# ambicuity/Distributed-LLM-Training-and-Inference-System

Measured on AMD Instinct MI355X. Metric: tokens/sec (node) GPT-7B train, higher is better.
Workload: dtype bf16; 1 GPU; model=gpt-7b, global_batch=16, seq_len=2048, parallelism=dp1, micro_batch=16, grad_accum=1, activation_checkpoint=none, layout=planner

## Files before the change

### llmctl/ops/csrc/flash_attn_bwd.hip

```cpp
#include <cstdlib>
#include <map>
#include <mutex>

#include "attn_common.h"

namespace llmctl {
using namespace attn;
namespace {

constexpr float LOG2E = 1.4426950408889634f;
constexpr int KV_KB = 128;
constexpr int KV_QT = 64;
#ifndef LLMCTL_DKV_NBUF
#define LLMCTL_DKV_NBUF 2
#endif
constexpr int KV_NBUF = LLMCTL_DKV_NBUF;
static_assert(KV_NBUF >= 2 && KV_NBUF <= 4, "dK/dV ring depth 2-4");
constexpr int DQ_QB = 128;
constexpr int DQ_KB = 64;

struct BwdArgs {
  const unsigned short *q, *k, *v, *dout;
  const float* lse;
  const float* delta;
// ... 264 lines not shown
#pragma unroll
        for (int d = 0; d < NDB; ++d) {
          dfr[d] = tr_frag<HD>(Ds, 32 * h, d * 32, lane);
          qfr[d] = tr_frag<HD>(Qs, 32 * h, d * 32, lane);
        }
      }
      __builtin_amdgcn_sched_barrier(0);
      if (need_mask) {
#pragma unroll
        for (int gq = 0; gq < 4; ++gq) {
          const int row0 = 32 * h + 8 * gq + 4 * hh;
          int sv[4] = {0, 0, 0, 0};
          if constexpr (DOC) {
            const int4 s4 = *reinterpret_cast<const int4*>(doc_s + row0);
            sv[0] = s4.x; sv[1] = s4.y; sv[2] = s4.z; sv[3] = s4.w;
          }
#pragma unroll
          for (int j = 0; j < 4; ++j) {
            const int qq = q0 + row0 + j;
            bool ok = qq < a.S && my_key < a.S;
            if constexpr (CAUSAL) ok = ok && my_key <= qq;
            if constexpr (DOC) ok = ok && my_key >= sv[j];
            s[4 * gq + j] = ok ? s[4 * gq + j] : -INFINITY;
          }
        }
      }
      float p[16], dsv[16];
#pragma unroll
      for (int i = 0; i < 16; ++i) {
        const float pv = fast_exp2(s[i] * a.scale_log2);
        p[i] = pv;
        dsv[i] = pv * dp[i];
      }
      bf16x8_t pb[2], sb[2];
      pb[0] = to_bf16x8(p);
      pb[1] = to_bf16x8(p + 8);
      sb[0] = to_bf16x8(dsv);
      sb[1] = to_bf16x8(dsv + 8);
      if constexpr (!CAUSAL) {
#pragma unroll
        for (int d = 0; d < NDB; ++d) {
          dfr[d] = tr_frag<HD>(Ds, 32 * h, d * 32, lane);
          qfr[d] = tr_frag<HD>(Qs, 32 * h, d * 32, lane);
        }
      }
      bf16x8_t dfr1[NDB], qfr1[NDB];
#pragma unroll
      for (int d = 0; d < NDB; ++d) {
        dfr1[d] = tr_frag<HD>(Ds, 32 * h + 16, d * 32, lane);
        qfr1[d] = tr_frag<HD>(Qs, 32 * h + 16, d * 32, lane);
      }
      dvdk_step<NDB>(dv, dk, dfr, qfr, pb[0], sb[0]);
      dvdk_step<NDB>(dv, dk, dfr1, qfr1, pb[1], sb[1]);
    }
  };
  for (int t = 0; t < ntiles; t += NB) {
    step(std::integral_constant<int, 0>{}, t);
    if (t + 1 < ntiles) step(std::integral_constant<int, 1>{}, t + 1);
    if constexpr (NB >= 3)
      if (t + 2 < ntiles) step(std::integral_constant<int, 2 % NB>{}, t + 2);
    if constexpr (NB >= 4)
      if (t + 3 < ntiles) step(std::integral_constant<int, 3 % NB>{}, t + 3);
  }
#pragma unroll
  for (int d = 0; d < NDB; ++d) asm volatile("s_nop 7\n\ts_nop 7" : "+a"(dk[d]), "+a"(dv[d]));
  if (my_key < a.S) {
    const long tok = (long)b * a.S + my_key;
    unsigned short* dkp = a.dk + tok * a.dk_st + (long)hk * HD;
    unsigned short* dvp = a.dv + tok * a.dv_st + (long)hk * HD;
    const float *cr = nullptr, *sr = nullptr;
    if (a.cos_t != nullptr) {
      const long p = a.rope_pos ? (long)a.rope_pos[tok] : tok % a.rope_S;
      cr = a.cos_t + p * (HD / 2);
      sr = a.sin_t + p * (HD / 2);
    }
    store_row<HD>(dkp, dk, a.scale, hh, cr, sr);
    store_row<HD>(dvp, dv, 1.f, hh, nullptr, nullptr);
  }
}

using s2_t = __attribute__((ext_vector_type(2))) unsigned int;

__device__ __forceinline__ bf16x8_t words8(unsigned w0, unsigned w1, unsigned w2, unsigned w3) {
  using u4 = __attribute__((ext_vector_type(4))) unsigned;
  return __builtin_bit_cast(bf16x8_t, u4{w0, w1, w2, w3});
}

__device__ __forceinline__ void mfma_v(f32x16& acc, bf16x8_t a, bf16x8_t b) {
  asm volatile("v_mfma_f32_32x32x16_bf16 %0, %1, %2, %0" : "+v"(acc) : "v"(a), "a"(b) : "memory");
}

__device__ __forceinline__ void x_step(f32x16& acc_s, f32x16& acc_d, bf16x8_t a_s, bf16x8_t b_s, bf16x8_t a_d,
                                       bf16x8_t b_d, float s0, float s1, float d0, float d1, float c, unsigned& pw,
                                       unsigned& dw) {
  float t0, t1, p0, p1;
  asm volatile(
      "v_mul_f32 %[t0], %[c], %[s0]\n\t"
      "v_mul_f32 %[t1], %[c], %[s1]\n\t"
      "v_mfma_f32_32x32x16_bf16 %[as], %[xs], %[ys], %[as]\n\t"
      "v_exp_f32 %[p0], %[t0]\n\t"
      "v_exp_f32 %[p1], %[t1]\n\t"
      "v_mfma_f32_32x32x16_bf16 %[ad], %[xd], %[yd], %[ad]\n\t"
      "v_mul_f32 %[t0], %[p0], %[d0]\n\t"
      "v_mul_f32 %[t1], %[p1], %[d1]\n\t"
      "v_cvt_pk_bf16_f32 %[pw], %[p0], %[p1]\n\t"
      "v_cvt_pk_bf16_f32 %[dw], %[t0], %[t1]"
      : [as] "+v"(acc_s), [ad] "+v"(acc_d), [t0] "=&v"(t0), [t1] "=&v"(t1), [p0] "=&v"(p0), [p1] "=&v"(p1),
        [pw] "=&v"(pw), [dw] "=&v"(dw)
      : [xs] "v"(a_s), [ys] "a"(b_s), [xd] "v"(a_d), [yd] "a"(b_d), [s0] "v"(s0), [s1] "v"(s1), [d0] "v"(d0),
        [d1] "v"(d1), [c] "s"(c)
      : "memory");
}

__device__ __forceinline__ void y_step(f32x16& dv, f32x16& dk, bf16x8_t da, bf16x8_t qa, bf16x8_t p, bf16x8_t ds,
                                       float s0, float s1, float d0, float d1, float c, unsigned& pw, unsigned& dw) {
  float t0, t1, p0, p1;
  asm volatile(
      "v_mul_f32 %[t0], %[c], %[s0]\n\t"
      "v_mul_f32 %[t1], %[c], %[s1]\n\t"
      "v_mfma_f32_32x32x16_bf16 %[dv], %[da], %[p], %[dv]\n\t"
      "v_exp_f32 %[p0], %[t0]\n\t"
      "v_exp_f32 %[p1], %[t1]\n\t"
      "v_mfma_f32_32x32x16_bf16 %[dk], %[qa], %[ds], %[dk]\n\t"
      "v_mul_f32 %[t0], %[p0], %[d0]\n\t"
      "v_mul_f32 %[t1], %[p1], %[d1]\n\t"
      "v_cvt_pk_bf16_f32 %[pw], %[p0], %[p1]\n\t"
      "v_cvt_pk_bf16_f32 %[dw], %[t0], %[t1]"
      : [dv] "+a"(dv), [dk] "+a"(dk), [t0] "=&v"(t0), [t1] "=&v"(t1), [p0] "=&v"(p0), [p1] "=&v"(p1),
        [pw] "=&v"(pw), [dw] "=&v"(dw)
      : [da] "v"(da), [qa] "v"(qa), [p] "v"(p), [ds] "v"(ds), [s0] "v"(s0), [s1] "v"(s1), [d0] "v"(d0),
        [d1] "v"(d1), [c] "s"(c)
      : "memory");
}

__device__ __forceinline__ f32x16 acc_copy(const f32x16& acc) {
  f32x16 out = acc;
  asm volatile("" : "+v"(out)::"memory");
  return out;
}
__device__ __forceinline__ void acc_zero(f32x16& acc) {
  const bf16x8_t z = {};
  asm volatile("s_nop 2\n\tv_mfma_f32_32x32x16_bf16 %0, %1, %1, 0" : "+a"(acc) : "v"(z));
}

__device__ __forceinline__ void z_step(f32x16& dv, f32x16& dk, bf16x8_t da, bf16x8_t qa, bf16x8_t p, bf16x8_t ds) {
  asm volatile(
      "v_mfma_f32_32x32x16_bf16 %[dv], %[da], %[p], %[dv]\n\t"
      "v_mfma_f32_32x32x16_bf16 %[dk], %[qa], %[ds], %[dk]"
      : [dv] "+a"(dv), [dk] "+a"(dk)
      : [da] "v"(da), [qa] "v"(qa), [p] "v"(p), [ds] "v"(ds)
      : "memory");
}

template <int HD, bool CAUSAL, bool DOC, bool STAMP = false>
__global__ __launch_bounds__(256, 1) void fa_bwd_dkv_pipe_kernel(BwdArgs a) {
  static_assert(HD == 128 && CAUSAL, "pipelined dK/dV kernel: causal, head_dim 128");
  constexpr int NKS = HD / 16;
  constexpr int NDB = HD / 32;
  constexpr int ROWB = HD * 2;
  constexpr int TILE_B = KV_QT * ROWB;
  constexpr int NP = TILE_B / 1024 / 4;
  constexpr int RC_B = KV_QT * 4;
  constexpr int BUF_B = 2 * TILE_B + 4 * RC_B;
  __shared__ __attribute__((aligned(1024))) unsigned char smem[2 * BUF_B];

  const int tid = threadIdx.x;
  const int lane = tid & 63;
  const int wave = __builtin_amdgcn_readfirstlane(tid >> 6);
  const int r = lane & 31, hh = lane >> 5;
  auto stamp = [&](int i) __attribute__((always_inline)) {
    if constexpr (STAMP) {
      if (tid == 0) a.stamps[blockIdx.x * 8 + i] = __builtin_amdgcn_s_memrealtime();
    }
  };
  stamp(0);
  if constexpr (STAMP) {
    if (tid == 0)
      a.stamps[blockIdx.x * 8 + 1] = (unsigned long long)(unsigned)__builtin_amdgcn_s_getreg(63492) |
                                     ((unsigned long long)(unsigned)__builtin_amdgcn_s_getreg(63508) << 32);
  }
  const int nkb = (a.S + KV_KB - 1) / KV_KB;
  const int BH = a.B * a.Hkv;
  int bh, kblk;
  if (BH % 8) {
    bh = blockIdx.x % BH;
    kblk = blockIdx.x / BH;
  } else {
    const int x = blockIdx.x & 7, j = blockIdx.x >> 3;
    bh = x * (BH >> 3) + j / nkb;
    kblk = j % nkb;
  }
  const int b = bh / a.Hkv, hk = bh % a.Hkv;
  const int group = a.Hq / a.Hkv;
  const int k0 = kblk * KV_KB;
  const int wkey0 = k0 + wave * 32;
  const int my_key = wkey0 + r;

  if (a.S % KV_QT) {
#pragma unroll
    for (int i = 0; i < 2 * BUF_B / 4096; ++i)
      *reinterpret_cast<uint4*>(smem + i * 4096 + tid * 16) = make_uint4(0, 0, 0, 0);
    if (tid < (2 * BUF_B % 4096) / 16)
      *reinterpret_cast<uint4*>(smem + (2 * BUF_B / 4096) * 4096 + tid * 16) = make_uint4(0, 0, 0, 0);
    __syncthreads();
  }

  const unsigned lds0 = lds_addr(smem);

  f32x16 dk[NDB], dv[NDB];
#pragma unroll
  for (int d = 0; d < NDB; ++d)
#pragma unroll
    for (int i = 0; i < 16; ++i) dk[d][i] = dv[d][i] = 0.f;

  const int q_start = CAUSAL ? k0 : 0;
  int q_end = a.S;
  if constexpr (DOC) {
    const int* ds = a.doc + (long)b * a.S;
    int lo = min(k0 + KV_KB, a.S), hi = a.S;
    while (lo < hi) {
      const int mid = (lo + hi) >> 1;
      if (ds[mid] > k0 + KV_KB - 1) hi = mid;
      else lo = mid + 1;
    }
    q_end = __builtin_amdgcn_readfirstlane(lo);
  }
  const int nq = q_end > q_start ? (q_end - q_start + KV_QT - 1) / KV_QT : 0;
  const int ntiles = group * nq;
  unsigned vq[NP], vd[NP];
#pragma unroll
  for (int i = 0; i < NP; ++i) {
    const int byte = (i * 4 + wave) * 1024 + lane * 16;
    const int row = byte / ROWB;
    const int lch = ((byte % ROWB) >> 4) ^ swz_tr<HD>(row);
    vq[i] = (unsigned)((row * a.q_ss + lch * 8) * 2);
    vd[i] = (unsigned)((row * a.do_ss + lch * 8) * 2);
  }
  const float* rc_src = a.rck_w + (wave == 1 ? a.rc_n : 0);
  const unsigned rc_off =
      (DOC && wave == 2) ? lane * 4
                         : (unsigned)((32 * (lane >> 5) + 8 * ((lane >> 2) & 3) + 4 * ((lane >> 4) & 1) + (lane & 3)) * 4);
  int iq0 = q_start;
  const unsigned short* qh = a.q + b * a.q_sb + (long)(hk * group) * a.q_sh;
  const unsigned short* dh = a.dout + b * a.do_sb + (long)(hk * group) * a.do_sh;
  const float* rh = rc_src + ((long)b * a.Hq + hk * group) * a.S;
  const unsigned short* qc = qh + (long)q_start * a.q_ss;
  const unsigned short* dc = dh + (long)q_start * a.do_ss;
  const long q_step = (long)KV_QT * a.q_ss, d_step = (long)KV_QT * a.do_ss;
  auto issue = [&](auto slot_c) __attribute__((always_inline)) {
    constexpr int SLC = decltype(slot_c)::value;
    const int nr = min(KV_QT, a.S - iq0);
    i32x4_t rq = buf_rsrc(qc, (unsigned)(((nr - 1) * a.q_ss + HD) * 2));
    i32x4_t rd = buf_rsrc(dc, (unsigned)(((nr - 1) * a.do_ss + HD) * 2));
    i32x4_t rr = (DOC && wave == 2) ? buf_rsrc(a.doc + (long)b * a.S + iq0, (unsigned)(nr * 4))
                                    : buf_rsrc(rh + iq0, (unsigned)(nr * 4));
    asm volatile("s_nop 4" : "+s"(rq), "+s"(rd), "+s"(rr));
    const unsigned slot = lds0 + (unsigned)(SLC * BUF_B);
#pragma unroll
    for (int i = 0; i < NP; ++i) {
      buf_dma16(rq, vq[i], slot + (i * 4 + wave) * 1024);
      buf_dma16(rd, vd[i], slot + TILE_B + (i * 4 + wave) * 1024);
    }
    buf_dma4(rr, rc_off, slot + 2 * TILE_B + wave * RC_B);
    iq0 += KV_QT;
    qc += q_step;
    dc += d_step;
    if (iq0 >= q_end) {
      iq0 = q_start;
      qh += a.q_sh;
      dh += a.do_sh;
      rh += a.S;
      qc = qh + (long)q_start * a.q_ss;
      dc = dh + (long)q_start * a.do_ss;
    }
  };

  const float c = a.scale_log2;
  auto apply_mask = [&](f32x16& s, int h, int q0, const int* doc_s) __attribute__((always_inline)) {
#pragma unroll
    for (int gq = 0; gq < 4; ++gq) {
      const int row0 = 32 * h + 8 * gq + 4 * hh;
      int sv[4] = {0, 0, 0, 0};
      if constexpr (DOC) {
        const int4 s4 = *reinterpret_cast<const int4*>(doc_s + row0);
        sv[0] = s4.x; sv[1] = s4.y; sv[2] = s4.z; sv[3] = s4.w;
      }
#pragma unroll
      for (int j = 0; j < 4; ++j) {
        const int qq = q0 + row0 + j;
        bool ok = qq < a.S && my_key < a.S;
        if constexpr (CAUSAL) ok = ok && my_key <= qq;
        if constexpr (DOC) ok = ok && my_key >= sv[j];
        s[4 * gq + j] = ok ? s[4 * gq + j] : -INFINITY;
      }
    }
  };

  if (ntiles > 0) issue(std::integral_constant<int, 0>{});
  bf16x8_t kf[NKS], vf[NKS];
  {
    const int kc = min(my_key, a.S - 1);
    const unsigned short* Kp = a.k + b * a.k_sb + hk * a.k_sh + (long)kc * a.k_ss + 8 * hh;
    const unsigned short* Vp = a.v + b * a.v_sb + hk * a.v_sh + (long)kc * a.v_ss + 8 * hh;
#pragma unroll
    for (int ks = 0; ks < NKS; ++ks) {
      asm volatile("global_load_dwordx4 %0, %1, off" : "=a"(kf[ks]) : "v"(Kp + 16 * ks) : "memory");
      asm volatile("global_load_dwordx4 %0, %1, off" : "=a"(vf[ks]) : "v"(Vp + 16 * ks) : "memory");
    }
  }
  vm_wait_n<0>();
  __builtin_amdgcn_s_barrier();
  stamp(2);
  if (ntiles > 1) issue(std::integral_constant<int, 1>{});
  int qi = 0;
  auto tile = [&](auto slot_c, int t) __attribute__((always_inline)) {
    constexpr int SL = decltype(slot_c)::value;
    const int q0 = q_start + qi * KV_QT;
    if (++qi == nq) qi = 0;
    const bool live = !(CAUSAL && wkey0 > q0 + KV_QT - 1);
    const unsigned char* Qs = smem + SL * BUF_B;
    const unsigned char* Ds = Qs + TILE_B;
    const float* lse_s = reinterpret_cast<const float*>(Ds + TILE_B);
    const float* del_s = lse_s + KV_QT;
    const int* doc_s = reinterpret_cast<const int*>(del_s + KV_QT);
    if (!live) return;
    f32x16 s0 = *reinterpret_cast<const f32x16*>(lse_s + 16 * hh);
    f32x16 p0 = *reinterpret_cast<const f32x16*>(del_s + 16 * hh);
    bf16x8_t qa[NKS], da[NKS];
#pragma unroll
    for (int ks = 0; ks < NKS; ++ks) {
      qa[ks] = lds_read_b128(Qs, tr_off<HD>(r, 2 * ks + hh));
      da[ks] = lds_read_b128(Ds, tr_off<HD>(r, 2 * ks + hh));
    }
    const bool need_mask = DOC || (CAUSAL && wkey0 + 31 > q0) || (q0 + KV_QT > a.S) || (wkey0 + 31 >= a.S);
#pragma unroll
    for (int ks = 0; ks < NKS; ++ks) {
      mfma_v(s0, qa[ks], kf[ks]);
      mfma_v(p0, da[ks], vf[ks]);
    }
    f32x16 s1 = *reinterpret_cast<const f32x16*>(lse_s + 32 + 16 * hh);
    f32x16 p1 = *reinterpret_cast<const f32x16*>(del_s + 32 + 16 * hh);
#pragma unroll
    for (int ks = 0; ks < NKS; ++ks) {
      qa[ks] = lds_read_b128(Qs, tr_off<HD>(32 + r, 2 * ks + hh));
      da[ks] = lds_read_b128(Ds, tr_off<HD>(32 + r, 2 * ks + hh));
    }
    if (need_mask) apply_mask(s0, 0, q0, doc_s);
    unsigned pw0[8], dw0[8];
    bf16x8_t td[2][NDB], tq[2][NDB];
#pragma unroll
    for (int ks = 0; ks < NKS; ++ks) {
      x_step(s1, p1, qa[ks], kf[ks], da[ks], vf[ks], s0[2 * ks], s0[2 * ks + 1], p0[2 * ks], p0[2 * ks + 1], c, pw0[ks],
             dw0[ks]);
      const int st = ks >> 2, d = ks & 3;
      td[st][d] = tr_frag<HD>(Ds, 16 * st, d * 32, lane);
      tq[st][d] = tr_frag<HD>(Qs, 16 * st, d * 32, lane);
    }
    if (need_mask) apply_mask(s1, 1, q0, doc_s);
    unsigned pw1[8], dw1[8];
    bf16x8_t cd[2][NDB], cq[2][NDB];
#pragma unroll
    for (int st = 0; st < 2; ++st) {
      const bf16x8_t pb = words8(pw0[4 * st], pw0[4 * st + 1], pw0[4 * st + 2], pw0[4 * st + 3]);
      const bf16x8_t sb = words8(dw0[4 * st], dw0[4 * st + 1], dw0[4 * st + 2], dw0[4 * st + 3]);
#pragma unroll
      for (int d = 0; d < NDB; ++d) {
        const int i = 4 * st + d;
        y_step(dv[d], dk[d], td[st][d], tq[st][d], pb, sb, s1[2 * i], s1[2 * i + 1], p1[2 * i], p1[2 * i + 1], c,
               pw1[i], dw1[i]);
        cd[st][d] = tr_frag<HD>(Ds, 32 + 16 * st, d * 32, lane);
        cq[st][d] = tr_frag<HD>(Qs, 32 + 16 * st, d * 32, lane);
      }
    }
#pragma unroll
    for (int st = 0; st < 2; ++st) {
      const bf16x8_t pb = words8(pw1[4 * st], pw1[4 * st + 1], pw1[4 * st + 2], pw1[4 * st + 3]);
      const bf16x8_t sb = words8(dw1[4 * st], dw1[4 * st + 1], dw1[4 * st + 2], dw1[4 * st + 3]);
#pragma unroll
      for (int d = 0; d < NDB; ++d) z_step(dv[d], dk[d], cd[st][d], cq[st][d], pb, sb);
    }
  };
  auto advance = [&](auto slot_c, int t) __attribute__((always_inline)) {
    constexpr int SL = decltype(slot_c)::value;
    asm volatile("s_waitcnt lgkmcnt(0)" ::: "memory");
    vm_wait_n<0>();
    __builtin_amdgcn_s_barrier();
    if (t + 2 < ntiles) issue(std::integral_constant<int, SL>{});
  };
  for (int t = 0; t < ntiles; t += 2) {
    tile(std::integral_constant<int, 0>{}, t);
    advance(std::integral_constant<int, 0>{}, t);
    if (t + 1 < ntiles) {
      tile(std::integral_constant<int, 1>{}, t + 1);
      advance(std::integral_constant<int, 1>{}, t + 1);
    }
  }
  stamp(3);
#pragma unroll
  for (int d = 0; d < NDB; ++d) asm volatile("s_nop 7\n\ts_nop 7" : "+a"(dk[d]), "+a"(dv[d]));
  if (my_key < a.S) {
    const long tok = (long)b * a.S + my_key;
    unsigned short* dkp = a.dk + tok * a.dk_st + (long)hk * HD;
    unsigned short* dvp = a.dv + tok * a.dv_st + (long)hk * HD;
    const float *cr = nullptr, *sr = nullptr;
    if (a.cos_t != nullptr) {
      const long p = a.rope_pos ? (long)a.rope_pos[tok] : tok % a.rope_S;
      cr = a.cos_t + p * (HD / 2);
      sr = a.sin_t + p * (HD / 2);
    }
    store_row<HD>(dkp, dk, a.scale, hh, cr, sr);
    store_row<HD>(dvp, dv, 1.f, hh, nullptr, nullptr);
  }
  if constexpr (STAMP) {
    asm volatile("s_waitcnt vmcnt(0)" ::: "memory");
    __syncthreads();
    stamp(4);
    if (tid == 0) a.stamps[blockIdx.x * 8 + 5] = (unsigned long long)ntiles;
  }
}

template <bool STAMP>
__global__ __launch_bounds__(256, 1) void fa_bwd_dkv_persist_kernel(BwdArgs a, int* __restrict__ wq) {
  constexpr int HD = 128;
  constexpr int NKS = HD / 16;
  constexpr int NDB = HD / 32;
  constexpr int ROWB = HD * 2;
  constexpr int TILE_B = KV_QT * ROWB;
  constexpr int NP = TILE_B / 1024 / 4;
  constexpr int RC_B = KV_QT * 4;
  constexpr int BUF_B = 2 * TILE_B + 4 * RC_B;
  __shared__ __attribute__((aligned(1024))) unsigned char smem[2 * BUF_B + 64];
  int* item_w = reinterpret_cast<int*>(smem + 2 * BUF_B);

  const int tid = threadIdx.x;
  const int lane = tid & 63;
  const int wave = __builtin_amdgcn_readfirstlane(tid >> 6);
  const int r = lane & 31, hh = lane >> 5;
  const int nkb = a.S / KV_KB;
  const int BH = a.B * a.Hkv;
  const bool per_xcd = BH % 8 == 0;
  const int xq = per_xcd ? (int)(blockIdx.x & 7) : 0;
  const int n_items = (per_xcd ? BH / 8 : BH) * nkb;
  const int bh_base = per_xcd ? xq * (BH / 8) : 0;
  const int group = a.Hq / a.Hkv;
  auto pop = [&]() __attribute__((always_inline)) -> int {
    const int j = __hip_atomic_fetch_add(wq + xq, 1, __ATOMIC_RELAXED, __HIP_MEMORY_SCOPE_AGENT);
    return j < n_items ? j : -1;
  };
  if (tid == 0) {
    const int i0 = pop();
    item_w[1] = i0;
    item_w[2] = i0 >= 0 ? pop() : -1;
  }
  __syncthreads();
  int cur = __builtin_amdgcn_readfirstlane(item_w[1]);
  int nxt = __builtin_amdgcn_readfirstlane(item_w[2]);
  if (cur < 0) return;

  const unsigned lds0 = lds_addr(smem);
  unsigned vq[NP], vd[NP];
#pragma unroll
  for (int i = 0; i < NP; ++i) {
    const int byte = (i * 4 + wave) * 1024 + lane * 16;
    const int row = byte / ROWB;
    const int lch = ((byte % ROWB) >> 4) ^ swz_tr<HD>(row);
    vq[i] = (unsigned)((row * a.q_ss + lch * 8) * 2);
    vd[i] = (unsigned)((row * a.do_ss + lch * 8) * 2);
  }
  const float* rc_src = a.rck_w + (wave == 1 ? a.rc_n : 0);
  const unsigned rc_off =
      (unsigned)((32 * (lane >> 5) + 8 * ((lane >> 2) & 3) + 4 * ((lane >> 4) & 1) + (lane & 3)) * 4);

  int iss = cur, iq0 = 0, iq_start = 0, ig = 0;
  const unsigned short *qh = nullptr, *dh = nullptr;
  const float* rh = nullptr;
  bool look_pending = false;
  int n_switch = 0;
  int pend0 = -1, pend1 = -1, npend = 0;
  auto iss_begin = [&](int item) __attribute__((always_inline)) {
    const int bh = bh_base + item / nkb, kb = item % nkb;
    const int bb = bh / a.Hkv, hkk = bh % a.Hkv;
    iq_start = kb * KV_KB;
    iq0 = iq_start;
    ig = 0;
    qh = a.q + bb * a.q_sb + (long)(hkk * group) * a.q_sh;
    dh = a.dout + bb * a.do_sb + (long)(hkk * group) * a.do_sh;
    rh = rc_src + ((long)bb * a.Hq + hkk * group) * a.S;
  };
  iss_begin(cur);
  auto issue = [&](auto slot_c) __attribute__((always_inline)) {
    constexpr int SLC = decltype(slot_c)::value;
    i32x4_t rq = buf_rsrc(qh + (long)iq0 * a.q_ss, (unsigned)(((KV_QT - 1) * a.q_ss + HD) * 2));
    i32x4_t rd = buf_rsrc(dh + (long)iq0 * a.do_ss, (unsigned)(((KV_QT - 1) * a.do_ss + HD) * 2));
    i32x4_t rr = buf_rsrc(rh + iq0, (unsigned)(KV_QT * 4));
    asm volatile("s_nop 4" : "+s"(rq), "+s"(rd), "+s"(rr));
    const unsigned slot = lds0 + (unsigned)(SLC * BUF_B);
#pragma unroll
    for (int i = 0; i < NP; ++i) {
      buf_dma16(rq, vq[i], slot + (i * 4 + wave) * 1024);
      buf_dma16(rd, vd[i], slot + TILE_B + (i * 4 + wave) * 1024);
    }
    buf_dma4(rr, rc_off, slot + 2 * TILE_B + wave * RC_B);
    iq0 += KV_QT;
    if (iq0 >= a.S) {
      if (++ig < group) {
        iq0 = iq_start;
        qh += a.q_sh;
        dh += a.do_sh;
        rh += a.S;
      } else {
        iss = nxt;
        if (iss >= 0) {
          iss_begin(iss);
          if (tid == 0) item_w[3 + (n_switch & 1)] = pop();
          look_pending = true;
          ++n_switch;
        }
        if (npend == 0) pend0 = iss;
        else pend1 = iss;
        ++npend;
      }
    }
  };

  bf16x8_t kf[NKS], vf[NKS];
  auto load_kv = [&](int item) __attribute__((always_inline)) {
    const int bh = bh_base + item / nkb, kb = item % nkb;
    const int bb = bh / a.Hkv, hkk = bh % a.Hkv;
    const int key = kb * KV_KB + wave * 32 + r;
    const unsigned short* Kp = a.k + bb * a.k_sb + hkk * a.k_sh + (long)key * a.k_ss + 8 * hh;
    const unsigned short* Vp = a.v + bb * a.v_sb + hkk * a.v_sh + (long)key * a.v_ss + 8 * hh;
#pragma unroll
    for (int ks = 0; ks < NKS; ++ks) {
      asm volatile("global_load_dwordx4 %0, %1, off" : "+a"(kf[ks]) : "v"(Kp + 16 * ks) : "memory");
      asm volatile("global_load_dwordx4 %0, %1, off" : "+a"(vf[ks]) : "v"(Vp + 16 * ks) : "memory");
    }
  };

  issue(std::integral_constant<int, 0>{});
  load_kv(cur);
  asm volatile("s_waitcnt vmcnt(0)"
               : "+a"(kf[0]), "+a"(kf[1]), "+a"(kf[2]), "+a"(kf[3]), "+a"(kf[4]), "+a"(kf[5]), "+a"(kf[6]),
                 "+a"(kf[7]), "+a"(vf[0]), "+a"(vf[1]), "+a"(vf[2]), "+a"(vf[3]), "+a"(vf[4]), "+a"(vf[5]),
                 "+a"(vf[6]), "+a"(vf[7])
               :
               : "memory");
  __builtin_amdgcn_s_barrier();
  issue(std::integral_constant<int, 1>{});
  f32x16 dk[NDB], dv[NDB];
#pragma unroll
  for (int d = 0; d < NDB; ++d) {
    const bf16x8_t z = {};
    asm volatile("s_nop 2\n\tv_mfma_f32_32x32x16_bf16 %0, %1, %1, 0" : "=a"(dk[d]) : "v"(z));
    asm volatile("v_mfma_f32_32x32x16_bf16 %0, %1, %1, 0" : "=a"(dv[d]) : "v"(z));
  }
  const float c = a.scale_log2;

  int n_done = 0;
  auto stamp = [&](int k) __attribute__((always_inline)) {
    if constexpr (STAMP) {
      if (tid == 0 && n_done < 64)
        a.stamps[(blockIdx.x * 64 + n_done) * 4 + k] = k == 3 ? (unsigned long long)cur : __builtin_amdgcn_s_memrealtime();
    }
  };
  for (;;) {
    stamp(0);
    stamp(3);
    const int bh = bh_base + cur / nkb, kb = cur % nkb;
    const int b = bh / a.Hkv, hk = bh % a.Hkv;
    const int k0 = kb * KV_KB;
    const int wkey0 = k0 + wave * 32;
    const int my_key = wkey0 + r;
    const int ntiles = group * ((a.S - k0) / KV_QT);
    int q0 = k0;
    auto apply_mask = [&](f32x16& s, int h) __attribute__((always_inline)) {
#pragma unroll
      for (int gq = 0; gq < 4; ++gq) {
        const int row0 = q0 + 32 * h + 8 * gq + 4 * hh;
#pragma unroll
        for (int j = 0; j < 4; ++j) s[4 * gq + j] = my_key <= row0 + j ? s[4 * gq + j] : -INFINITY;
      }
    };
    auto tile = [&](auto slot_c) __attribute__((always_inline)) {
      constexpr int SL = decltype(slot_c)::value;
      const bool live = !(wkey0 > q0 + KV_QT - 1);
      if (!live) return;
      const unsigned char* Qs = smem + SL * BUF_B;
      const unsigned char* Ds = Qs + TILE_B;
      const float* lse_s = reinterpret_cast<const float*>(Ds + TILE_B);
      const float* del_s = lse_s + KV_QT;
      const bool need_mask = wkey0 + 31 > q0;
      f32x16 s0 = *reinterpret_cast<const f32x16*>(lse_s + 16 * hh);
      f32x16 p0 = *reinterpret_cast<const f32x16*>(del_s + 16 * hh);
      bf16x8_t qa[NKS], da[NKS];
#pragma unroll
      for (int ks = 0; ks < NKS; ++ks) {
        qa[ks] = lds_read_b128(Qs, tr_off<HD>(r, 2 * ks + hh));
        da[ks] = lds_read_b128(Ds, tr_off<HD>(r, 2 * ks + hh));
      }
      f32x16 s1 = *reinterpret_cast<const f32x16*>(lse_s + 32 + 16 * hh);
      f32x16 p1 = *reinterpret_cast<const f32x16*>(del_s + 32 + 16 * hh);
      bf16x8_t qb[NKS], db[NKS];
#pragma unroll
      for (int ks = 0; ks < NKS; ++ks) {
        mfma_v(s0, qa[ks], kf[ks]);
        qb[ks] = lds_read_b128(Qs, tr_off<HD>(32 + r, 2 * ks + hh));
        mfma_v(p0, da[ks], vf[ks]);
        db[ks] = lds_read_b128(Ds, tr_off<HD>(32 + r, 2 * ks + hh));
      }
      if (need_mask) apply_mask(s0, 0);
      unsigned pw0[8], dw0[8];
      bf16x8_t td[2][NDB], tq[2][NDB];
#pragma unroll
      for (int ks = 0; ks < NKS; ++ks) {
        x_step(s1, p1, qb[ks], kf[ks], db[ks], vf[ks], s0[2 * ks], s0[2 * ks + 1], p0[2 * ks], p0[2 * ks + 1], c,
               pw0[ks], dw0[ks]);
        const int st = ks >> 2, d = ks & 3;
        td[st][d] = tr_frag<HD>(Ds, 16 * st, d * 32, lane);
        tq[st][d] = tr_frag<HD>(Qs, 16 * st, d * 32, lane);
      }
      if (need_mask) apply_mask(s1, 1);
      unsigned pw1[8], dw1[8];
      bf16x8_t cd[2][NDB], cq[2][NDB];
#pragma unroll
      for (int st = 0; st < 2; ++st) {
        const bf16x8_t pb = words8(pw0[4 * st], pw0[4 * st + 1], pw0[4 * st + 2], pw0[4 * st + 3]);
        const bf16x8_t sb = words8(dw0[4 * st], dw0[4 * st + 1], dw0[4 * st + 2], dw0[4 * st + 3]);
#pragma unroll
        for (int d = 0; d < NDB; ++d) {
          const int i = 4 * st + d;
          y_step(dv[d], dk[d], td[st][d], tq[st][d], pb, sb, s1[2 * i], s1[2 * i + 1], p1[2 * i], p1[2 * i + 1], c,
                 pw1[i], dw1[i]);
          cd[st][d] = tr_frag<HD>(Ds, 32 + 16 * st, d * 32, lane);
          cq[st][d] = tr_frag<HD>(Qs, 32 + 16 * st, d * 32, lane);
        }
      }
#pragma unroll
      for (int st = 0; st < 2; ++st) {
        const bf16x8_t pb = words8(pw1[4 * st], pw1[4 * st + 1], pw1[4 * st + 2], pw1[4 * st + 3]);
        const bf16x8_t sb = words8(dw1[4 * st], dw1[4 * st + 1], dw1[4 * st + 2], dw1[4 * st + 3]);
#pragma unroll
        for (int d = 0; d < NDB; ++d) z_step(dv[d], dk[d], cd[st][d], cq[st][d], pb, sb);
      }
    };
    auto advance = [&](auto slot_c) __attribute__((always_inline)) {
      constexpr int SL = decltype(slot_c)::value;
      asm volatile("s_waitcnt lgkmcnt(0)" ::: "memory");
      vm_wait_n<0>();
      __builtin_amdgcn_s_barrier();
      if (look_pending) {
        nxt = __builtin_amdgcn_readfirstlane(item_w[3 + ((n_switch - 1) & 1)]);
        look_pending = false;
      }
      if (iss >= 0) issue(std::integral_constant<int, SL>{});
      q0 += KV_QT;
      if (q0 >= a.S) q0 = k0;
    };
    for (int t = 0; t < ntiles; t += 2) {
      tile(std::integral_constant<int, 0>{});
      advance(std::integral_constant<int, 0>{});
      tile(std::integral_constant<int, 1>{});
      advance(std::integral_constant<int, 1>{});
    }
    stamp(1);
    {
      const long tok = (long)b * a.S + my_key;
      unsigned short* dkp = a.dk + tok * a.dk_st + (long)hk * HD;
      unsigned short* dvp = a.dv + tok * a.dv_st + (long)hk * HD;
      const bool rope = a.cos_t != nullptr;
      f32x4 cs[NDB / 2][4], sn[NDB / 2][4];
      if (rope) {
        const long p = a.rope_pos ? (long)a.rope_pos[tok] : tok % a.rope_S;
        const float* cr = a.cos_t + p * (HD / 2);
        const float* sr = a.sin_t + p * (HD / 2);
#pragma unroll
        for (int d = 0; d < NDB / 2; ++d)
#pragma unroll
          for (int g = 0; g < 4; ++g) {
            const int col = d * 32 + 8 * g + 4 * hh;
            cs[d][g] = *reinterpret_cast<const f32x4*>(cr + col);
            sn[d][g] = *reinterpret_cast<const f32x4*>(sr + col);
          }
      }
#pragma unroll
      for (int d = 0; d < NDB; ++d) asm volatile("s_nop 7\n\ts_nop 7" : "+a"(dk[d]), "+a"(dv[d]));
      auto st8 = [&](unsigned short* p, const float* x, float mul) __attribute__((always_inline)) {
        s2_t w;
        w[0] = (unsigned)f2bf(x[0] * mul) | ((unsigned)f2bf(x[1] * mul) << 16);
        w[1] = (unsigned)f2bf(x[2] * mul) | ((unsigned)f2bf(x[3] * mul) << 16);
        asm volatile("global_store_dwordx2 %0, %1, off" ::"v"(p), "v"(w) : "memory");
      };
#pragma unroll
      for (int d = 0; d < NDB / 2; ++d) {
        const f32x16 x1 = acc_copy(dk[d]), x2 = acc_copy(dk[d + NDB / 2]);
        acc_zero(dk[d]);
        acc_zero(dk[d + NDB / 2]);
#pragma unroll
        for (int g = 0; g < 4; ++g) {
          const int col = d * 32 + 8 * g + 4 * hh;
          float lo[4], hi[4];
#pragma unroll
          for (int j = 0; j < 4; ++j) {
            const float c1 = rope ? cs[d][g][j] : 1.f, s1 = rope ? sn[d][g][j] : 0.f;
            lo[j] = x1[4 * g + j] * c1 + x2[4 * g + j] * s1;
            hi[j] = x2[4 * g + j] * c1 - x1[4 * g + j] * s1;
          }
          st8(dkp + col, lo, a.scale);
          st8(dkp + col + HD / 2, hi, a.scale);
        }
      }
#pragma unroll
      for (int d = 0; d < NDB; ++d) {
        const f32x16 x = acc_copy(dv[d]);
        acc_zero(dv[d]);
#pragma unroll
        for (int g = 0; g < 4; ++g) {
          float y[4];
#pragma unroll
          for (int j = 0; j < 4; ++j) y[j] = x[4 * g + j];
          st8(dvp + d * 32 + 8 * g + 4 * hh, y, 1.f);
        }
      }
      load_kv(pend0 >= 0 ? pend0 : cur);
      asm volatile("s_waitcnt vmcnt(0)"
                   : "+a"(kf[0]), "+a"(kf[1]), "+a"(kf[2]), "+a"(kf[3]), "+a"(kf[4]), "+a"(kf[5]), "+a"(kf[6]),
                     "+a"(kf[7]), "+a"(vf[0]), "+a"(vf[1]), "+a"(vf[2]), "+a"(vf[3]), "+a"(vf[4]), "+a"(vf[5]),
                     "+a"(vf[6]), "+a"(vf[7])
                   :
                   : "memory");
    }
    stamp(2);
    ++n_done;
    if (pend0 < 0) break;
    cur = pend0;
    pend0 = pend1;
    pend1 = -1;
    --npend;
  }
}

template <int HD, bool CAUSAL, bool DOC>
__global__ __launch_bounds__(256, 2) void fa_bwd_dq_kernel(BwdArgs a) {
  constexpr int NKS = HD / 16;
  constexpr int NDB = HD / 32;
  constexpr int ROWB = HD * 2;
  constexpr int TILE = DQ_KB * ROWB;
  constexpr int PPW = TILE / 1024 / 4;
  constexpr int SLOT = 2 * TILE;
  __shared__ __attribute__((aligned(1024))) unsigned char smem[2 * SLOT];

  const int tid = threadIdx.x;
  const int lane = tid & 63;
  const int wave = __builtin_amdgcn_readfirstlane(tid >> 6);
  const int r = lane & 31, hh = lane >> 5;
  const int nqb = (a.S + DQ_QB - 1) / DQ_QB;
  const int BH = a.B * a.Hq;
  int bh, qi;
  if (BH % 8) {
    bh = blockIdx.x % BH;
    qi = blockIdx.x / BH;
  } else {
    const int x = blockIdx.x & 7, j = blockIdx.x >> 3;
    bh = x * (BH >> 3) + j / nqb;
    qi = j % nqb;
  }
  const int qblk = nqb - 1 - qi;
  const int b = bh / a.Hq, hq = bh % a.Hq;
  const int hk = hq / (a.Hq / a.Hkv);
  const int q_row0 = qblk * DQ_QB + wave * 32;
  const int my_q = q_row0 + r;
  const int qc = min(my_q, a.S - 1);

  const unsigned short* Kp = a.k + b * a.k_sb + hk * a.k_sh;
  const unsigned short* Vp = a.v + b * a.v_sb + hk * a.v_sh;

#pragma unroll
  for (int i = 0; i < 2 * SLOT / 4096; ++i)
    *reinterpret_cast<uint4*>(smem + i * 4096 + tid * 16) = make_uint4(0, 0, 0, 0);

  bf16x8_t qf[NKS], df[NKS];
  {
    const unsigned short* Qp = a.q + b * a.q_sb + hq * a.q_sh + (long)qc * a.q_ss + 8 * hh;
    const unsigned short* Dp = a.dout + b * a.do_sb + hq * a.do_sh + (long)qc * a.do_ss + 8 * hh;
#pragma unroll
    for (int ks = 0; ks < NKS; ++ks) {
      qf[ks] = __builtin_bit_cast(bf16x8_t, gload16(Qp + 16 * ks));
      df[ks] = __builtin_bit_cast(bf16x8_t, gload16(Dp + 16 * ks));
    }
  }
  const long rc = ((long)b * a.Hq + hq) * a.S + qc;
  const float nlse2 = -a.lse[rc] * LOG2E;
  float dlt;
  if (a.o != nullptr) {
    const unsigned short* Op = a.o + b * a.o_sb + hq * a.o_sh + (long)qc * a.o_ss + 8 * hh;
    float acc = 0.f;
#pragma unroll
    for (int ks = 0; ks < NKS; ++ks) {
      const bf16x8_t of = __builtin_bit_cast(bf16x8_t, gload16(Op + 16 * ks));
#pragma unroll
      for (int j = 0; j < 8; ++j) acc += (float)of[j] * (float)df[ks][j];
    }
    dlt = xor32_add(acc);
    if (hh == 0 && my_q < a.S) a.delta_w[rc] = dlt;
  } else {
    dlt = a.delta[rc];
  }
  if (hh == 0 && my_q < a.S) {
// ... 360 lines not shown
```

Baseline: 31060 tokens/s.

## Interleave next-tile DMA and softmax math into MFMA stream in persistent dK/dV kernel

Rewrites the persistent flash-attention dK/dV backward tile loop so the prefetch of the next Q/dO/LSE tile is issued as separate buffer-to-LDS loads spread between the MFMAs of the current tile, instead of as one burst after the barrier. Softmax exp/scale/convert work is hand-scheduled in inline asm alongside the MFMAs. LDS fragment loads are software-pipelined one or two steps ahead, and transposed-fragment offsets are precomputed. Buffer descriptors use a zero range when no work remains, and the per-tile dead-tile early return is removed. This is meant to hide memory latency and VALU work behind matrix instructions, at the cost of more register pressure and a fragile hand-written instruction order.

```diff
diff --git a/llmctl/ops/csrc/flash_attn_bwd.hip b/llmctl/ops/csrc/flash_attn_bwd.hip
--- a/llmctl/ops/csrc/flash_attn_bwd.hip
+++ b/llmctl/ops/csrc/flash_attn_bwd.hip
@@ -440,6 +440,59 @@
       : "memory");
 }
 
+#define LLMCTL_SM_A_ASM                                        \
+  "v_mfma_f32_32x32x16_bf16 %[acc], %[fa], %[fb], %[acc]\n\t" \
+  "v_exp_f32 %[e0], %[t0]\n\t"                                 \
+  "v_exp_f32 %[e1], %[t1]\n\t"                                 \
+  "v_mul_f32 %[u0], %[e0], %[d0]"
+#define LLMCTL_SM_B_ASM                                        \
+  "v_mfma_f32_32x32x16_bf16 %[acc], %[fa], %[fb], %[acc]\n\t" \
+  "v_mul_f32 %[u1], %[e1], %[d1]\n\t"                          \
+  "v_cvt_pk_bf16_f32 %[pw], %[e0], %[e1]\n\t"                  \
+  "v_cvt_pk_bf16_f32 %[dw], %[u0], %[u1]"
+#define LLMCTL_SM_NEXT_ASM              \
+  "\n\tv_mul_f32 %[n0], %[c], %[s0]\n\t" \
+  "v_mul_f32 %[n1], %[c], %[s1]"
+
+__device__ __forceinline__ void sm_first(float& t0, float& t1, float c, float s0, float s1) {
+  asm volatile("v_mul_f32 %[n0], %[c], %[s0]\n\tv_mul_f32 %[n1], %[c], %[s1]"
+               : [n0] "=&v"(t0), [n1] "=&v"(t1)
+               : [c] "s"(c), [s0] "v"(s0), [s1] "v"(s1)
+               : "memory");
+}
+#define LLMCTL_SM_STEPS(PFX, ACC, FB)                                                                             \
+  __device__ __forceinline__ void PFX##a(f32x16& acc, bf16x8_t fa, bf16x8_t fb, float t0, float t1, float d0,     \
+                                         float& e0, float& e1, float& u0) {                                       \
+    asm volatile(LLMCTL_SM_A_ASM                                                                                  \
+                 : [acc] ACC(acc), [e0] "=&v"(e0), [e1] "=&v"(e1), [u0] "=&v"(u0)                                 \
+                 : [fa] "v"(fa), [fb] FB(fb), [t0] "v"(t0), [t1] "v"(t1), [d0] "v"(d0)                            \
+                 : "memory");                                                                                     \
+  }                                                                                                               \
+  __device__ __forceinline__ void PFX##b(f32x16& acc, bf16x8_t fa, bf16x8_t fb, float e0, float e1, float u0,     \
+                                         float d1, unsigned& pw, unsigned& dw, float c, float s0, float s1,       \
+                                         float& n0, float& n1) {                                                  \
+    float u1;                                                                                                     \
+    asm volatile(LLMCTL_SM_B_ASM LLMCTL_SM_NEXT_ASM                                                               \
+                 : [acc] ACC(acc), [u1] "=&v"(u1), [pw] "=&v"(pw), [dw] "=&v"(dw), [n0] "=&v"(n0), [n1] "=&v"(n1) \
+                 : [fa] "v"(fa), [fb] FB(fb), [e0] "v"(e0), [e1] "v"(e1), [u0] "v"(u0), [d1] "v"(d1), [c] "s"(c), \
+                   [s0] "v"(s0), [s1] "v"(s1)                                                                     \
+                 : "memory");                                                                                     \
+  }                                                                                                               \
+  __device__ __forceinline__ void PFX##b_last(f32x16& acc, bf16x8_t fa, bf16x8_t fb, float e0, float e1,          \
+                                              float u0, float d1, unsigned& pw, unsigned& dw) {                   \
+    float u1;                                                                                                     \
+    asm volatile(LLMCTL_SM_B_ASM                                                                                  \
+                 : [acc] ACC(acc), [u1] "=&v"(u1), [pw] "=&v"(pw), [dw] "=&v"(dw)                                 \
+                 : [fa] "v"(fa), [fb] FB(fb), [e0] "v"(e0), [e1] "v"(e1), [u0] "v"(u0), [d1] "v"(d1)              \
+                 : "memory");                                                                                     \
+  }
+LLMCTL_SM_STEPS(x, "+v", "a")
+LLMCTL_SM_STEPS(y, "+a", "v")
+#undef LLMCTL_SM_STEPS
+#undef LLMCTL_SM_A_ASM
+#undef LLMCTL_SM_B_ASM
+#undef LLMCTL_SM_NEXT_ASM
+
 template <int HD, bool CAUSAL, bool DOC, bool STAMP = false>
 __global__ __launch_bounds__(256, 1) void fa_bwd_dkv_pipe_kernel(BwdArgs a) {
   static_assert(HD == 128 && CAUSAL, "pipelined dK/dV kernel: causal, head_dim 128");
@@ -707,6 +760,18 @@
   }
 }
 
+template <int OFF>
+__device__ __forceinline__ void buf_dma16_off(i32x4_t rsrc, unsigned voff, unsigned lds_base) {
+  asm volatile("s_add_u32 m0, %2, %3\n\ts_nop 0\n\tbuffer_load_dwordx4 %0, %1, 0 offen lds" ::"v"(voff), "s"(rsrc),
+               "s"(lds_base), "i"(OFF)
+               : "memory", "scc");
+}
+template <int OFF>
+__device__ __forceinline__ void buf_dma4_off(i32x4_t rsrc, unsigned voff, unsigned lds_base) {
+  asm volatile("s_add_u32 m0, %2, %3\n\ts_nop 0\n\tbuffer_load_dword %0, %1, 0 offen lds" ::"v"(voff), "s"(rsrc),
+               "s"(lds_base), "i"(OFF)
+               : "memory", "scc");
+}
 template <bool STAMP>
 __global__ __launch_bounds__(256, 1) void fa_bwd_dkv_persist_kernel(BwdArgs a, int* __restrict__ wq) {
   constexpr int HD = 128;
@@ -758,10 +823,17 @@
   const float* rc_src = a.rck_w + (wave == 1 ? a.rc_n : 0);
   const unsigned rc_off =
       (unsigned)((32 * (lane >> 5) + 8 * ((lane >> 2) & 3) + 4 * ((lane >> 4) & 1) + (lane & 3)) * 4);
+  int tlo[NDB], thi[NDB];
+#pragma unroll
+  for (int d = 0; d < NDB; ++d) tr_frag_offs<HD>(d * 32, lane, tlo[d], thi[d]);
+  const unsigned lds_w = lds0 + (unsigned)(wave * 1024), lds_rc = lds0 + (unsigned)(wave * RC_B);
 
   int iss = cur, iq0 = 0, iq_start = 0, ig = 0;
-  const unsigned short *qh = nullptr, *dh = nullptr;
-  const float* rh = nullptr;
+  const unsigned short *qc = nullptr, *dc = nullptr;
+  const float* rc = nullptr;
+  long q_wrap = 0, d_wrap = 0;
+  const long q_step = (long)KV_QT * a.q_ss, d_step = (long)KV_QT * a.do_ss;
+  const unsigned q_rec = (unsigned)(((KV_QT - 1) * a.q_ss + HD) * 2), d_rec = (unsigned)(((KV_QT - 1) * a.do_ss + HD) * 2);
   bool look_pending = false;
   int n_switch = 0;
   int pend0 = -1, pend1 = -1, npend = 0;
@@ -771,31 +843,33 @@
     iq_start = kb * KV_KB;
     iq0 = iq_start;
     ig = 0;
-    qh = a.q + bb * a.q_sb + (long)(hkk * group) * a.q_sh;
-    dh = a.dout + bb * a.do_sb + (long)(hkk * group) * a.do_sh;
-    rh = rc_src + ((long)bb * a.Hq + hkk * group) * a.S;
+    qc = a.q + bb * a.q_sb + (long)(hkk * group) * a.q_sh + (long)iq_start * a.q_ss;
+    dc = a.dout + bb * a.do_sb + (long)(hkk * group) * a.do_sh + (long)iq_start * a.do_ss;
+    rc = rc_src + ((long)bb * a.Hq + hkk * group) * a.S + iq_start;
+    q_wrap = a.q_sh - (long)(a.S - iq_start) * a.q_ss;
+    d_wrap = a.do_sh - (long)(a.S - iq_start) * a.do_ss;
   };
   iss_begin(cur);
-  auto issue = [&](auto slot_c) __attribute__((always_inline)) {
-    constexpr int SLC = decltype(slot_c)::value;
-    i32x4_t rq = buf_rsrc(qh + (long)iq0 * a.q_ss, (unsigned)(((KV_QT - 1) * a.q_ss + HD) * 2));
-    i32x4_t rd = buf_rsrc(dh + (long)iq0 * a.do_ss, (unsigned)(((KV_QT - 1) * a.do_ss + HD) * 2));
-    i32x4_t rr = buf_rsrc(rh + iq0, (unsigned)(KV_QT * 4));
+  i32x4_t rq, rd, rr;
+  auto iss_desc = [&]() __attribute__((always_inline)) {
+    const bool on = iss >= 0;
+    rq = buf_rsrc(qc, on ? q_rec : 0u);
+    rd = buf_rsrc(dc, on ? d_rec : 0u);
+    rr = buf_rsrc(rc, on ? (unsigned)(KV_QT * 4) : 0u);
     asm volatile("s_nop 4" : "+s"(rq), "+s"(rd), "+s"(rr));
-    const unsigned slot = lds0 + (unsigned)(SLC * BUF_B);
-#pragma unroll
-    for (int i = 0; i < NP; ++i) {
-      buf_dma16(rq, vq[i], slot + (i * 4 + wave) * 1024);
-      buf_dma16(rd, vd[i], slot + TILE_B + (i * 4 + wave) * 1024);
-    }
-    buf_dma4(rr, rc_off, slot + 2 * TILE_B + wave * RC_B);
+  };
+  auto iss_next = [&]() __attribute__((always_inline)) {
+    if (iss < 0) return;
     iq0 += KV_QT;
+    qc += q_step;
+    dc += d_step;
+    rc += KV_QT;
     if (iq0 >= a.S) {
       if (++ig < group) {
         iq0 = iq_start;
-        qh += a.q_sh;
-        dh += a.do_sh;
-        rh += a.S;
+        qc += q_wrap;
+        dc += d_wrap;
+        rc += iq_start;
       } else {
         iss = nxt;
         if (iss >= 0) {
@@ -810,6 +884,24 @@
       }
     }
   };
+  static_assert(NP == 4 && TILE_B == 4 * 4096, "pieces per tile and wave");
+  auto iss_piece = [&](auto slot_c, int j) __attribute__((always_inline)) {
+    constexpr int SO = decltype(slot_c)::value * BUF_B;
+    if (j == 0) buf_dma16_off<SO>(rq, vq[0], lds_w);
+    else if (j == 1) buf_dma16_off<SO + TILE_B>(rd, vd[0], lds_w);
+    else if (j == 2) buf_dma16_off<SO + 4096>(rq, vq[1], lds_w);
+    else if (j == 3) buf_dma16_off<SO + TILE_B + 4096>(rd, vd[1], lds_w);
+    else if (j == 4) buf_dma16_off<SO + 8192>(rq, vq[2], lds_w);
+    else if (j == 5) buf_dma16_off<SO + TILE_B + 8192>(rd, vd[2], lds_w);
+    else if (j == 6) buf_dma16_off<SO + 12288>(rq, vq[3], lds_w);
+    else if (j == 7) buf_dma16_off<SO + TILE_B + 12288>(rd, vd[3], lds_w);
+    else if (j == 8) buf_dma4_off<SO + 2 * TILE_B>(rr, rc_off, lds_rc);
+  };
+  auto issue = [&](auto slot_c) __attribute__((always_inline)) {
+    iss_desc();
+#pragma unroll
+    for (int j = 0; j < 9; ++j) iss_piece(slot_c, j);
+  };
 
   bf16x8_t kf[NKS], vf[NKS];
   auto load_kv = [&](int item) __attribute__((always_inline)) {
@@ -826,6 +918,7 @@
   };
 
   issue(std::integral_constant<int, 0>{});
+  iss_next();
   load_kv(cur);
   asm volatile("s_waitcnt vmcnt(0)"
                : "+a"(kf[0]), "+a"(kf[1]), "+a"(kf[2]), "+a"(kf[3]), "+a"(kf[4]), "+a"(kf[5]), "+a"(kf[6]),
@@ -834,7 +927,6 @@
                :
                : "memory");
   __builtin_amdgcn_s_barrier();
-  issue(std::integral_constant<int, 1>{});
   f32x16 dk[NDB], dv[NDB];
 #pragma unroll
   for (int d = 0; d < NDB; ++d) {
@@ -871,57 +963,93 @@
     };
     auto tile = [&](auto slot_c) __attribute__((always_inline)) {
       constexpr int SL = decltype(slot_c)::value;
-      const bool live = !(wkey0 > q0 + KV_QT - 1);
-      if (!live) return;
       const unsigned char* Qs = smem + SL * BUF_B;
       const unsigned char* Ds = Qs + TILE_B;
       const float* lse_s = reinterpret_cast<const float*>(Ds + TILE_B);
       const float* del_s = lse_s + KV_QT;
       const bool need_mask = wkey0 + 31 > q0;
+      const auto rc4 = [&](const float* p, int i) __attribute__((always_inline)) {
+        return *reinterpret_cast<const f32x4*>(p + 16 * hh + 4 * i);
+      };
+      const auto cat16 = [](f32x4 x0, f32x4 x1, f32x4 x2, f32x4 x3) __attribute__((always_inline)) {
+        return f32x16{x0[0], x0[1], x0[2], x0[3], x1[0], x1[1], x1[2], x1[3],
+                      x2[0], x2[1], x2[2], x2[3], x3[0], x3[1], x3[2], x3[3]};
+      };
+      bf16x8_t qa[NKS], da[NKS], qb[NKS], db[NKS];
       f32x16 s0 = *reinterpret_cast<const f32x16*>(lse_s + 16 * hh);
+      qa[0] = lds_read_b128(Qs, tr_off<HD>(r, hh));
+      asm volatile("" ::: "memory");
       f32x16 p0 = *reinterpret_cast<const f32x16*>(del_s + 16 * hh);
-      bf16x8_t qa[NKS], da[NKS];
-#pragma unroll
-      for (int ks = 0; ks < NKS; ++ks) {
-        qa[ks] = lds_read_b128(Qs, tr_off<HD>(r, 2 * ks + hh));
-        da[ks] = lds_read_b128(Ds, tr_off<HD>(r, 2 * ks + hh));
-      }
-      f32x16 s1 = *reinterpret_cast<const f32x16*>(lse_s + 32 + 16 * hh);
-      f32x16 p1 = *reinterpret_cast<const f32x16*>(del_s + 32 + 16 * hh);
-      bf16x8_t qb[NKS], db[NKS];
+      da[0] = lds_read_b128(Ds, tr_off<HD>(r, hh));
+      asm volatile("" ::: "memory");
+      qa[1] = lds_read_b128(Qs, tr_off<HD>(r, 2 + hh));
+      da[1] = lds_read_b128(Ds, tr_off<HD>(r, 2 + hh));
+      qa[2] = lds_read_b128(Qs, tr_off<HD>(r, 4 + hh));
+      da[2] = lds_read_b128(Ds, tr_off<HD>(r, 4 + hh));
+      iss_desc();
+      f32x4 s1q[4], p1q[4];
+      auto s_slot = [&](int j) __attribute__((always_inline)) {
+        const int ks = j >> 1, e = j - 4;
+        if (ks + 3 < NKS) {
+          if (j & 1) da[ks + 3] = lds_read_b128(Ds, tr_off<HD>(r, 2 * (ks + 3) + hh));
+          else qa[ks + 3] = lds_read_b128(Qs, tr_off<HD>(r, 2 * (ks + 3) + hh));
+        }
+        if (e >= 0 && e < 4) s1q[e] = rc4(lse_s + 32, e);
+        else if (e >= 4 && e < 8) p1q[e - 4] = rc4(del_s + 32, e - 4);
+        else if (e == 8) qb[0] = lds_read_b128(Qs, tr_off<HD>(32 + r, hh));
+        else if (e == 9) db[0] = lds_read_b128(Ds, tr_off<HD>(32 + r, hh));
+        else if (e == 10) qb[1] = lds_read_b128(Qs, tr_off<HD>(32 + r, 2 + hh));
+        else if (e == 11) db[1] = lds_read_b128(Ds, tr_off<HD>(32 + r, 2 + hh));
+        if (j < 4) iss_piece(std::integral_constant<int, 1 - SL>{}, j);
+        else if (j >= 10 && j < 15) iss_piece(std::integral_constant<int, 1 - SL>{}, j - 6);
+      };
 #pragma unroll
       for (int ks = 0; ks < NKS; ++ks) {
         mfma_v(s0, qa[ks], kf[ks]);
-        qb[ks] = lds_read_b128(Qs, tr_off<HD>(32 + r, 2 * ks + hh));
+        s_slot(2 * ks);
         mfma_v(p0, da[ks], vf[ks]);
-        db[ks] = lds_read_b128(Ds, tr_off<HD>(32 + r, 2 * ks + hh));
-      }
+        s_slot(2 * ks + 1);
+      }
+      f32x16 s1 = cat16(s1q[0], s1q[1], s1q[2], s1q[3]);
+      f32x16 p1 = cat16(p1q[0], p1q[1], p1q[2], p1q[3]);
       if (need_mask) apply_mask(s0, 0);
       unsigned pw0[8], dw0[8];
       bf16x8_t td[2][NDB], tq[2][NDB];
+      float t0, t1;
+      sm_first(t0, t1, c, s0[0], s0[1]);
 #pragma unroll
       for (int ks = 0; ks < NKS; ++ks) {
-        x_step(s1, p1, qb[ks], kf[ks], db[ks], vf[ks], s0[2 * ks], s0[2 * ks + 1], p0[2 * ks], p0[2 * ks + 1], c,
-               pw0[ks], dw0[ks]);
         const int st = ks >> 2, d = ks & 3;
-        td[st][d] = tr_frag<HD>(Ds, 16 * st, d * 32, lane);
-        tq[st][d] = tr_frag<HD>(Qs, 16 * st, d * 32, lane);
+        float e0, e1, u0;
+        xa(s1, qb[ks], kf[ks], t0, t1, p0[2 * ks], e0, e1, u0);
+        td[st][d] = tr_frag_at<HD>(Ds, 16 * st, tlo[d], thi[d]);
+        if (ks + 2 < NKS) qb[ks + 2] = lds_read_b128(Qs, tr_off<HD>(32 + r, 2 * (ks + 2) + hh));
+        if (ks + 1 < NKS)
+          xb(p1, db[ks], vf[ks], e0, e1, u0, p0[2 * ks + 1], pw0[ks], dw0[ks], c, s0[(2 * ks + 2) & 15],
+             s0[(2 * ks + 3) & 15], t0, t1);
+        else
+          xb_last(p1, db[ks], vf[ks], e0, e1, u0, p0[2 * ks + 1], pw0[ks], dw0[ks]);
+        tq[st][d] = tr_frag_at<HD>(Qs, 16 * st, tlo[d], thi[d]);
+        if (ks + 2 < NKS) db[ks + 2] = lds_read_b128(Ds, tr_off<HD>(32 + r, 2 * (ks + 2) + hh));
       }
       if (need_mask) apply_mask(s1, 1);
       unsigned pw1[8], dw1[8];
       bf16x8_t cd[2][NDB], cq[2][NDB];
-#pragma unroll
-      for (int st = 0; st < 2; ++st) {
+      sm_first(t0, t1, c, s1[0], s1[1]);
+#pragma unroll
+      for (int i = 0; i < 2 * NDB; ++i) {
+        const int st = i / NDB, d = i % NDB;
         const bf16x8_t pb = words8(pw0[4 * st], pw0[4 * st + 1], pw0[4 * st + 2], pw0[4 * st + 3]);
         const bf16x8_t sb = words8(dw0[4 * st], dw0[4 * st + 1], dw0[4 * st + 2], dw0[4 * st + 3]);
-#pragma unroll
-        for (int d = 0; d < NDB; ++d) {
-          const int i = 4 * st + d;
-          y_step(dv[d], dk[d], td[st][d], tq[st][d], pb, sb, s1[2 * i], s1[2 * i + 1], p1[2 * i], p1[2 * i + 1], c,
-                 pw1[i], dw1[i]);
-          cd[st][d] = tr_frag<HD>(Ds, 32 + 16 * st, d * 32, lane);
-          cq[st][d] = tr_frag<HD>(Qs, 32 + 16 * st, d * 32, lane);
-        }
+        float e0, e1, u0;
+        ya(dv[d], td[st][d], pb, t0, t1, p1[2 * i], e0, e1, u0);
+        cd[st][d] = tr_frag_at<HD>(Ds, 32 + 16 * st, tlo[d], thi[d]);
+        if (i + 1 < 2 * NDB)
+          yb(dk[d], tq[st][d], sb, e0, e1, u0, p1[2 * i + 1], pw1[i], dw1[i], c, s1[(2 * i + 2) & 15],
+             s1[(2 * i + 3) & 15], t0, t1);
+        else
+          yb_last(dk[d], tq[st][d], sb, e0, e1, u0, p1[2 * i + 1], pw1[i], dw1[i]);
+        cq[st][d] = tr_frag_at<HD>(Qs, 32 + 16 * st, tlo[d], thi[d]);
       }
 #pragma unroll
       for (int st = 0; st < 2; ++st) {
@@ -940,7 +1068,7 @@
         nxt = __builtin_amdgcn_readfirstlane(item_w[3 + ((n_switch - 1) & 1)]);
         look_pending = false;
       }
-      if (iss >= 0) issue(std::integral_constant<int, SL>{});
+      iss_next();
       q0 += KV_QT;
       if (q0 >= a.S) q0 = k0;
     };
```

Measured after the change: 31280 tokens/s (median of 6 runs). Within noise of the previous version (+0.7%).
